# HopperLogger/HopperRender

Hardware: AMD Instinct MI355X
Metric: interpolated frames/sec + ms/flow-calc, 2160p HDR, 1/2/4/8 MI355X (higher is better)
Workload: dtype u16

## Files before the change

### hopperrender_amd/calc.py

```python
import ctypes as C

import numpy as np

from . import capi

BlendedFrame = 2
WarpedFrame12, WarpedFrame21, HSVFlow, GreyFlow, SideBySide1, SideBySide2 = 0, 1, 3, 4, 5, 6


def _ptr(a):
    if isinstance(a, np.ndarray):
        if not a.flags["C_CONTIGUOUS"]:
            raise ValueError("frame buffers must be C-contiguous")
        return a.ctypes.data_as(C.c_void_p)
    return C.c_void_p(a)


class OpticalFlowCalc:

    is_hdr = False

    def __init__(self, frameHeight, frameWidth, inputStride=0, outputStride=0, deltaScalar=8, neighborScalar=6,
                 blackLevel=0.0, whiteLevel=255.0, maxCalcRes=270, *, device_index=0, iterations=0, blur_radius=0,
                 search_radius=0, flags=0):
# ... 197 lines not shown
        return ms.value

    def profile(self):
        pr = capi.HfProfile()
        capi.check(self._lib.hf_get_profile(self._ctx, C.byref(pr)), self._ctx)
        return {k: getattr(pr, k) for k, _ in pr._fields_}

    def setProfileInterval(self, warp_every, flow_every):
        capi.check(self._lib.hf_set_profile_interval(self._ctx, int(warp_every), int(flow_every)), self._ctx)

    def resetProfile(self):
        capi.check(self._lib.hf_reset_profile(self._ctx), self._ctx)

    def readOffsets(self):
        a = np.empty((2, self.m_opticalFlowFrameHeight, self.m_opticalFlowFrameWidth), dtype=np.int16)
        capi.check(self._lib.hf_read_offsets(self._ctx, _ptr(a)), self._ctx)
        return a

    def readBlurredFlow(self, idx):
        a = np.empty((2, self.m_opticalFlowFrameHeight, self.m_opticalFlowFrameWidth), dtype=np.int16)
        capi.check(self._lib.hf_read_blurred_flow(self._ctx, idx, _ptr(a)), self._ctx)
        return a

    def readPhasePlane(self, ring_slot):
        import ctypes
        n = int(self.phase_plane_bytes)
        a = np.empty(n // 4, dtype=np.uint32)
        done = ctypes.c_int(0)
        capi.check(self._lib.hf_read_phase_plane(self._ctx, ring_slot, _ptr(a), ctypes.byref(done)), self._ctx)
        return a, bool(done.value)

    def writeBlurredFlow(self, idx, flow):
        a = np.ascontiguousarray(flow, dtype=np.int16)
        assert a.shape == (2, self.m_opticalFlowFrameHeight, self.m_opticalFlowFrameWidth)
        capi.check(self._lib.hf_write_blurred_flow(self._ctx, idx, _ptr(a)), self._ctx)

    def deviceRcp(self, values):
        x = np.ascontiguousarray(values, dtype=np.float32)
        y = np.empty_like(x)
        capi.check(self._lib.hf_device_rcp(self._ctx, _ptr(x), _ptr(y), len(x)), self._ctx)
        return y

    def countersEnable(self, on=True):
        capi.check(self._lib.hf_debug_counters_enable(self._ctx, 1 if on else 0), self._ctx)

    def counters(self, reset=False):
        cc = capi.HfDebugCounters()
        capi.check(self._lib.hf_debug_counters_read(self._ctx, C.byref(cc), 1 if reset else 0), self._ctx)
        lv = {}
        for k in range(16):
            if cc.level_window_size[k] and (cc.level_windows[k][0] or cc.level_windows[k][1]):
                lv[int(cc.level_window_size[k])] = {"X": (int(cc.level_windows[k][0]), int(cc.level_reused[k][0])),
                                                     "Y": (int(cc.level_windows[k][1]), int(cc.level_reused[k][1]))}
        return {"warp_workgroups": dict(zip(("staged", "interior_global", "generic"), [int(x) for x in cc.warp_workgroups])), "levels": lv}

    def stats(self):
        s = self._stats()
        return {k: getattr(s, k) for k, _ in s._fields_}

    def close(self):
        if getattr(self, "_ctx", None):
            self._lib.hf_destroy(self._ctx)
            self._ctx = C.c_void_p()

    def __del__(self):
        try:
            self.close()
        except Exception:
            pass


class OpticalFlowCalcSDR(OpticalFlowCalc):
    is_hdr = False


class OpticalFlowCalcHDR(OpticalFlowCalc):
    is_hdr = True


ERROR_TILE_DTYPE = np.dtype([("sse", "<u8"), ("sad", "<u4"), ("max_abs", "<u4")])


def frame_error_maps(raw, n, tiles_x, tiles_y):
    a = np.ascontiguousarray(np.frombuffer(raw, dtype=np.uint8) if isinstance(raw, (bytes, bytearray, memoryview)) else raw).reshape(-1).view(np.uint8)
    need = n * 3 * tiles_y * tiles_x * ERROR_TILE_DTYPE.itemsize
    if a.size < need:
        raise ValueError(f"frame_error_maps: {a.size} bytes, {n} maps of 3 x {tiles_y} x {tiles_x} tiles need {need}")
    return a[:need].view(ERROR_TILE_DTYPE).reshape(n, 3, tiles_y, tiles_x)


class DeviceBuffer:

    def __init__(self, nbytes, device_index=0):
        self._lib = capi.load()
        self.device_index, self.nbytes = device_index, nbytes
        p = C.c_void_p()
        capi.check(self._lib.hf_device_malloc(device_index, nbytes, C.byref(p)))
        self.ptr = p.value

    def upload(self, a):
        a = np.ascontiguousarray(a)
        assert a.nbytes <= self.nbytes
        capi.check(self._lib.hf_memcpy_h2d(self.device_index, C.c_void_p(self.ptr), _ptr(a), a.nbytes))

    def download(self, dtype, count=None):
        dt = np.dtype(dtype)
        n = count if count is not None else self.nbytes // dt.itemsize
# ... 154 lines not shown
```

### hopperrender_amd/capi.py

```python
import ctypes as C
import os

from . import build as _build

HF_FLAG_ASYNC = 0x1
HF_FLAG_NO_GRAPH = 0x2
HF_FLAG_PROFILE = 0x4
HF_FLAG_NO_LAZY_ARGMIN = 0x8
HF_FLAG_DUAL_STREAM = 0x40
HF_FLAG_NO_FUSED_WARP = 0x80
HF_FLAG_NO_TIMING = 0x200
HF_FLAG_BATCH_NORMAL_PRIORITY = 0x800
HF_FLAG_BATCH_EAGER_PLANES = 0x1000
HF_FLAG_NO_SAD_REUSE = 0x2000
HF_FLAG_SAD_REUSE_ALWAYS = 0x4000
HF_FLAG_PLANAR_IN = 0x8000
HF_FLAG_PLANAR_OUT = 0x10000
HF_FLAG_BATCH_PLANAR_IN = 0x20000
HF_FLAG_BATCH_PLANAR_OUT = 0x40000
HF_FLAG_BATCH_AUTO_DEFERRED = 0x80000
HF_MAX_PERIOD_OUTPUTS = 6
HF_MAX_PERIOD_OUTPUTS_WIDE = 24
HF_MAX_ERROR_PAIRS = 192
HF_ERROR_SLOTS = 256
# ... 22 lines not shown
                ("first_output", C.c_int64), ("n_outputs", C.c_int64), ("blend_at_start", C.c_double)]


class HfHostioConfig(C.Structure):
    _fields_ = [("struct_size", C.c_uint32), ("in_ring", C.c_int32), ("out_ring", C.c_int32), ("frame_output_mode", C.c_int32),
                ("scene_change_threshold", C.c_int32), ("reserved", C.c_int32), ("source_frame_time", C.c_int64),
                ("target_frame_time", C.c_int64)]


HF_HOSTIO_FILL_FN = C.CFUNCTYPE(C.c_int, C.c_void_p, C.c_int64, C.c_void_p)
HF_HOSTIO_SINK_FN = C.CFUNCTYPE(C.c_int, C.c_void_p, C.c_int64, C.c_void_p, C.c_int32)


class HfParams(C.Structure):
    _fields_ = [("delta_scalar", C.c_int32), ("neighbor_scalar", C.c_int32), ("black_level", C.c_float),
                ("white_level", C.c_float), ("search_radius", C.c_int32), ("frame_count", C.c_uint32)]


class HfStats(C.Structure):
    _fields_ = [("total_frame_delta", C.c_uint32), ("frame_count", C.c_uint32), ("ofc_calc_time", C.c_double),
                ("ofc_avg_calc_time", C.c_double), ("ofc_peak_calc_time", C.c_double), ("warp_calc_time", C.c_double),
                ("res_scalar", C.c_int32), ("low_width", C.c_int32), ("low_height", C.c_int32),
                ("frame_width", C.c_int32), ("frame_height", C.c_int32), ("input_stride", C.c_int32),
                ("output_stride", C.c_int32), ("iterations", C.c_int32), ("initial_window", C.c_int32),
                ("input_frame_bytes", C.c_uint64), ("output_frame_bytes", C.c_uint64), ("phase_plane_bytes", C.c_uint64),
                ("sad_tables", C.c_int32), ("still_share", C.c_float)]


class HfTimelineRecord(C.Structure):
    _fields_ = [("kernel", C.c_char * 32), ("period", C.c_int32), ("flags", C.c_int32), ("start_ms", C.c_double), ("end_ms", C.c_double),
                ("duration_ms", C.c_double)]


class HfSceneRecord(C.Structure):
    _fields_ = [("frame_count", C.c_uint32), ("total_delta", C.c_uint32), ("kind", C.c_int32), ("average", C.c_int32), ("d1", C.c_int32),
                ("d2", C.c_int32)]


class HfFrameError(C.Structure):
    _fields_ = [("sse", C.c_uint64 * 3), ("sad", C.c_uint64 * 3), ("n_differ", C.c_uint64 * 3), ("count", C.c_uint64 * 3),
                ("max_abs", C.c_uint32 * 3), ("reserved", C.c_uint32)]


class HfFrameSsim(C.Structure):
    _fields_ = [("sum_loss_q32", C.c_uint64 * 3), ("max_loss_q32", C.c_uint64 * 3), ("count", C.c_uint64 * 3)]


class HfErrorTile(C.Structure):
    _fields_ = [("sse", C.c_uint64), ("sad", C.c_uint32), ("max_abs", C.c_uint32)]


class HfDebugCounters(C.Structure):
    _fields_ = [("warp_workgroups", C.c_uint32 * 3), ("reserved", C.c_uint32), ("level_windows", (C.c_uint32 * 2) * 16),
                ("level_reused", (C.c_uint32 * 2) * 16), ("level_window_size", C.c_int32 * 16)]


class HfLiveResources(C.Structure):
    _fields_ = [("device_buffers", C.c_int64), ("pinned_buffers", C.c_int64), ("streams", C.c_int64), ("events", C.c_int64),
                ("graph_execs", C.c_int64)]


class HfProfile(C.Structure):
    _fields_ = [("warp_launches", C.c_uint64), ("warp_ms", C.c_double), ("copy_launches", C.c_uint64),
                ("copy_ms", C.c_double), ("flow_chains", C.c_uint64), ("flow_ms", C.c_double), ("warp_frames", C.c_uint64)]


class HfFilterConfig(C.Structure):
    _fields_ = [("struct_size", C.c_uint32), ("scene_change_threshold", C.c_int32), ("source_frame_time", C.c_int64),
                ("target_frame_time", C.c_int64), ("frame_output_mode", C.c_int32), ("auto_adjust", C.c_int32),
                ("active", C.c_int32), ("reserved", C.c_int32)]


class HfFilterState(C.Structure):
    _fields_ = [("num_int_frames", C.c_int32), ("active", C.c_int32), ("blending_scalar", C.c_double),
                ("total_warp_duration", C.c_double), ("playback_frame_time", C.c_int64),
                ("peak_scene_change_delta", C.c_uint32), ("peak_scene_change_delta2", C.c_uint32),
                ("frame_delta_history", C.c_uint32), ("scene_change_history", C.c_uint32),
                ("average_frame_delta", C.c_int32), ("scene_change_delta1", C.c_int32), ("scene_change_delta2", C.c_int32)]


_vp, _i, _f = C.c_void_p, C.c_int, C.c_float
SIGNATURES = {
    "hf_create": (_i, [C.POINTER(HfConfig), C.POINTER(_vp)]),
    "hf_destroy": (None, [_vp]),
    "hf_last_error": (C.c_char_p, [_vp]),
    "hf_abi_version": (_i, []),
    "hf_select_device": (_i, [C.POINTER(HfDeviceCaps), _i, C.c_uint64, C.c_char_p, C.c_size_t]),
    "hf_get_device": (_i, [_vp]),
    "hf_update_frame": (_i, [_vp, _vp]),
    "hf_calculate_optical_flow": (_i, [_vp]),
    "hf_warp_frames": (_i, [_vp, _f, _i]),
    "hf_copy_frame": (_i, [_vp]),
    "hf_download_frame": (_i, [_vp, _vp]),
    "hf_get_params": (_i, [_vp, C.POINTER(HfParams)]),
    "hf_set_params": (_i, [_vp, C.POINTER(HfParams)]),
    "hf_get_stats": (_i, [_vp, C.POINTER(HfStats)]),
    "hf_update_frame_device": (_i, [_vp, _vp]),
    "hf_update_frame_device_ref": (_i, [_vp, _vp]),
    "hf_update_frame_async": (_i, [_vp, _vp]),
    "hf_download_frame_async": (_i, [_vp, _vp]),
    "hf_wait_flow": (_i, [_vp]),
    "hf_downloads_issued": (C.c_uint64, [_vp]),
    "hf_wait_download": (_i, [_vp, C.c_uint64]),
    "hf_interpolate_period": (_i, [_vp, _vp, _i, C.POINTER(C.c_float), C.POINTER(_vp), _i]),
    "hf_interpolate_period_ex": (_i, [_vp, _vp, _i, C.POINTER(C.c_float), C.POINTER(_vp), _i, _i]),
    "hf_batch_create": (_i, [C.POINTER(_vp), _i, C.POINTER(_vp)]),
    "hf_batch_destroy": (None, [_vp]),
# ... 169 lines not shown
```

### hopperrender_amd/csrc/hf_context.hip

```cpp

#include "hf_ctx.h"

using namespace hfi;

namespace {
thread_local std::string g_create_error;
}

namespace hfi {
std::shared_mutex g_capture_mutex;
std::atomic<int64_t> g_live[kLiveKinds];
}

namespace hfi {

int fail(hf_ctx* c, int code, const char* fmt, ...) {
    char buf[512];
    va_list ap;
    va_start(ap, fmt);
    vsnprintf(buf, sizeof(buf), fmt, ap);
    va_end(ap);
    std::string msg = std::string("[HopperRender] ") + buf;
    if (c) c->err = msg; else g_create_error = msg;
    return code;
// ... 409 lines not shown
    if (int rc = set_device(c)) return rc;
    if (int rc = sync_ctx(c)) return rc;
    HF_HIP(c, hipMemcpyAsync(c->blurred[idx].get(), host_in, 2 * c->plane_elems * sizeof(int16_t), hipMemcpyHostToDevice, c->stream));
    hf::launch_pack_flow(c->g, c->blurred[idx].get(), c->blurred_xy[idx].get(), c->stream);
    HF_HIP(c, hipStreamSynchronize(c->stream));
    return HF_OK;
}

int hf_timer_begin(hf_ctx* c) {
    HF_CHECK_CTX(c);
    if (int rc = set_device(c)) return rc;
    if (int rc = leave_warp_stream(c)) return rc;
    HF_HIP(c, hipEventRecord(c->ev_user0.get(), c->stream));
    return HF_OK;
}

int hf_timer_end(hf_ctx* c, float* elapsed_ms) {
    HF_CHECK_CTX(c);
    if (!elapsed_ms) return fail(c, HF_ERR_INVALID_ARGUMENT, "hf_timer_end: null");
    if (int rc = set_device(c)) return rc;
    if (int rc = leave_warp_stream(c)) return rc;
    HF_HIP(c, hipEventRecord(c->ev_user1.get(), c->stream));
    HF_HIP(c, hipEventSynchronize(c->ev_user1.get()));
    HF_HIP(c, hipEventElapsedTime(elapsed_ms, c->ev_user0.get(), c->ev_user1.get()));
    return HF_OK;
}

int hf_debug_counters_enable(hf_ctx* c, int on) {
    HF_CHECK_CTX(c);
    if (int rc = set_device(c)) return rc;
    if (int rc = sync_ctx(c)) return rc;
    c->graphs.clear();
    if (c->batch) c->batch->graphs.clear();
    if (on) {
        if (!c->counters) HF_HIP(c, alloc_device(c->counters, hf::kCounterWords * sizeof(uint32_t)));
        HF_HIP(c, hipMemsetAsync(c->counters.get(), 0, hf::kCounterWords * sizeof(uint32_t), c->stream));
        return sync_ctx(c);
    }
    c->counters.reset();
    return HF_OK;
}

int hf_debug_counters_read(hf_ctx* c, hf_debug_counters* out, int reset) {
    HF_CHECK_CTX(c);
    if (!out) return fail(c, HF_ERR_INVALID_ARGUMENT, "hf_debug_counters_read: null");
    if (!c->counters) return fail(c, HF_ERR_STATE, "hf_debug_counters_read: hf_debug_counters_enable(ctx, 1) first");
    if (int rc = set_device(c)) return rc;
    if (int rc = sync_ctx(c)) return rc;
    uint32_t w[hf::kCounterWords];
    HF_HIP(c, hipMemcpy(w, c->counters.get(), sizeof(w), hipMemcpyDeviceToHost));
    if (reset) HF_HIP(c, hipMemset(c->counters.get(), 0, sizeof(w)));
    memset(out, 0, sizeof(*out));
    for (int i = 0; i < 3; i++) out->warp_workgroups[i] = w[hf::kCounterWarp + i];
    for (int k = 0; k < 16; k++) {
        for (int ax = 0; ax < 2; ax++) {
            out->level_windows[k][ax] = w[hf::kCounterLevels + 4 * k + 2 * ax];
            out->level_reused[k][ax] = w[hf::kCounterLevels + 4 * k + 2 * ax + 1];
        }
        out->level_window_size[k] = k < (int)c->levels.size() && k < c->last_iterations ? c->levels[(size_t)k].window : 0;
    }
    return HF_OK;
}

int hf_debug_bounds_violations(hf_ctx* c, uint32_t* count, uint32_t first[4], int reset) {
    if (!c || !count) return HF_ERR_INVALID_ARGUMENT;
    if (int rc = set_device(c)) return rc;
    if (hipDeviceSynchronize() != hipSuccess) return fail(c, HF_ERR_HIP, "hf_debug_bounds_violations: hipDeviceSynchronize failed");
    unsigned rec[5] = {0, 0, 0, 0, 0};
    const bool a = hf::dbg_bounds_read_kernels(rec, reset != 0), b = hf::dbg_bounds_read_flow(rec, reset != 0),
               p = hf::dbg_bounds_read_planar(rec, reset != 0), s = hf::dbg_bounds_read_scene(rec, reset != 0),
               m = hf::dbg_bounds_read_metrics(rec, reset != 0);
    if (!a || !b || !p || !s || !m) return fail(c, HF_ERR_STATE, "hf_debug_bounds_violations: this library was built without -DHF_DEBUG_BOUNDS (python -m hopperrender_amd.build --debug-bounds)");
    *count = rec[0];
    if (first) for (int i = 0; i < 4; i++) first[i] = rec[1 + i];
    return HF_OK;
}

int hf_debug_bounds_selftest(hf_ctx* c) {
    if (!c) return HF_ERR_INVALID_ARGUMENT;
    uint32_t before = 0, after = 0, first[4] = {0, 0, 0, 0};
    if (int rc = hf_debug_bounds_violations(c, &before, nullptr, 0)) return rc;
    DevBuf<int> scratch;
    if (alloc_device(scratch, 80 * sizeof(int)) != hipSuccess) return fail(c, HF_ERR_OUT_OF_MEMORY, "hf_debug_bounds_selftest: hipMalloc failed");
    hf::launch_bounds_selftest(scratch.get(), c->stream);
    if (hipStreamSynchronize(c->stream) != hipSuccess) return fail(c, HF_ERR_HIP, "hf_debug_bounds_selftest: launch failed");
    if (int rc = hf_debug_bounds_violations(c, &after, first, 0)) return rc;
    if (after - before != 64u || (before == 0 && first[0] != 999u))
        return fail(c, HF_ERR_STATE, "hf_debug_bounds_selftest: 64 out-of-range indices were issued, %u recorded (first site %u)", after - before, first[0]);
    return HF_OK;
}

int hf_device_rcp(hf_ctx* c, const float* host_in, float* host_out, int n) {
    HF_CHECK_CTX(c);
    if (!host_in || !host_out || n < 1 || n > 32) return fail(c, HF_ERR_INVALID_ARGUMENT, "hf_device_rcp: bad argument");
    if (int rc = set_device(c)) return rc;
    if (int rc = sync_ctx(c)) return rc;
    HF_HIP(c, hipMemcpyAsync(c->d_probe.get(), host_in, n * sizeof(float), hipMemcpyHostToDevice, c->stream));
    hf::launch_rcp_probe(c->d_probe.get(), c->d_probe.get() + 32, n, c->stream);
    HF_HIP(c, hipMemcpyAsync(host_out, c->d_probe.get() + 32, n * sizeof(float), hipMemcpyDeviceToHost, c->stream));
    HF_HIP(c, hipStreamSynchronize(c->stream));
    return HF_OK;
}

__global__ void clock_probe_kernel(unsigned long long ticks, unsigned long long* out) {
    const unsigned long long r0 = __builtin_amdgcn_s_memrealtime(), c0 = __builtin_amdgcn_s_memtime();
    unsigned long long r1 = r0;
// ... 95 lines not shown
```

### hopperrender_amd/csrc/hf_kernels.hip

```cpp
#include "hf_kernels.h"
#include "hf_phase_plane.h"
#include "hf_levels.h"
#include <type_traits>

#include <hip/hip_ext.h>

namespace hf {

namespace {

__device__ __forceinline__ int clampi(int v, int lo, int hi) { return min(max(v, lo), hi); }
typedef unsigned nt_uint4 __attribute__((ext_vector_type(4)));
__device__ __forceinline__ void store16_streaming(void* dst, const void* src16) {
    __builtin_nontemporal_store(*(const nt_uint4*)src16, (nt_uint4*)dst);
}
__device__ __forceinline__ unsigned absdiff(unsigned a, unsigned b) { return a > b ? a - b : b - a; }

__device__ __forceinline__ int rel_offset(int layer, int R) {
    const int d = layer - (R >> 1);
    return d > 0 ? d * d : -(d * d);
}

__device__ __forceinline__ int mirror_flow(int pos, int dim) {
    if (pos >= dim) pos = 2 * dim - pos - 1; else if (pos < 0) pos = -pos - 1;
// ... 779 lines not shown
    const int chunk = u % n_chunks, v = u / n_chunks;
    const int member = v / n_blocks, blk = v - member * n_blocks;
    const WarpArgs& a = batch.s[member];
    const int ti0 = chunk * out_chunk, ti1 = min(a.n_out, ti0 + out_chunk);
    if (ti0 >= ti1) return;
    const int tile = blk * wpb + __builtin_amdgcn_readfirstlane(threadIdx.x >> 6);
    if (tile >= n_tiles) return;
    const int trow = tile / wpr, tcol = tile - trow * wpr;
    const int lane = threadIdx.x & 63;
    const int cx0 = (tcol * kWarpTX + (lane & (kWarpTX - 1))) * VEC;
    if (cx0 >= g.W) return;
    if (trow >= y_tiles) {
        const int rg = (trow - y_tiles) * kWarpTY + (lane / kWarpTX);
        if (rg < uv_groups) warp_fast_body<E, GROUP, ROWS, MODE, 1, VB, DW>(g, a, rg * ROWS, cx0, ti0, ti1);
    } else {
        const int rg = trow * kWarpTY + (lane / kWarpTX);
        if (rg < y_groups) warp_fast_body<E, GROUP, ROWS, MODE, 0, VB, DW>(g, a, rg * ROWS, cx0, ti0, ti1);
    }
}


typedef unsigned short ushort2w __attribute__((ext_vector_type(2)));
template <bool MAX>
__device__ __forceinline__ uint32_t pk_mm_u16(uint32_t a, uint32_t b) {
    ushort2w x, y;
    __builtin_memcpy(&x, &a, 4); __builtin_memcpy(&y, &b, 4);
    const ushort2w m = MAX ? __builtin_elementwise_max(x, y) : __builtin_elementwise_min(x, y);
    uint32_t r;
    __builtin_memcpy(&r, &m, 4);
    return r;
}
template <int CTRL>
__device__ __forceinline__ uint32_t dpp_mov(uint32_t v) { return (uint32_t)__builtin_amdgcn_update_dpp(0, (int)v, CTRL, 0xF, 0xF, true); }
template <bool MAX>
__device__ __forceinline__ uint32_t wave_pk_mm_u16(uint32_t v) {
    v = pk_mm_u16<MAX>(v, dpp_mov<0xB1>(v));
    v = pk_mm_u16<MAX>(v, dpp_mov<0x4E>(v));
    v = pk_mm_u16<MAX>(v, dpp_mov<0x141>(v));
    v = pk_mm_u16<MAX>(v, dpp_mov<0x140>(v));
    const uint32_t r0 = (uint32_t)__builtin_amdgcn_readlane((int)v, 0), r1 = (uint32_t)__builtin_amdgcn_readlane((int)v, 16),
                   r2 = (uint32_t)__builtin_amdgcn_readlane((int)v, 32), r3 = (uint32_t)__builtin_amdgcn_readlane((int)v, 48);
    return pk_mm_u16<MAX>(pk_mm_u16<MAX>(r0, r1), pk_mm_u16<MAX>(r2, r3));
}

constexpr int kExtX = 64, kExtY = 64;
constexpr int kWgCells = 64;

template <int NW>
struct WgShared {
    uint2 tab[kMaxWarpOutputs][kWgCells];
    uint32_t bounds[NW][4];
    int state[NW];
    int item[NW];
};

template <typename E, int MODE, int CZ, int NW, int ROWS>
__device__ __forceinline__ void warp_wg_body(const Geom& g, const WarpArgs& a, const int tx0, const int ty0, const bool lane_valid, const int wave,
                                             unsigned char* const lds, WgShared<NW>& sh, uint32_t* const counters) {
    constexpr int VEC = 16 / (int)sizeof(E), NDW = 4, CHUNKS = wg_chunks(NW * ROWS / 2), SZ = (int)sizeof(E);
    constexpr int TW = kWarpTX * VEC, TH = NW * kWarpTY * ROWS, NT = 64 * NW;
    constexpr bool need_a = MODE != 1, need_b = MODE != 0;
    const int H = g.H, W = g.W, Si = g.in_stride, So = g.out_stride, rs = g.rs, lw = g.lw, lh = g.lh;
    const int dim_y = CZ ? (H >> 1) : H;
    const int n = a.n_out;
    const unsigned tid = threadIdx.x, lane = tid & 63u;
    const int cx0 = tx0 + (int)(lane & (kWarpTX - 1)) * VEC, cy0 = ty0 + (wave * kWarpTY + (int)(lane / kWarpTX)) * ROWS;
    const uint64_t valid_mask = __builtin_amdgcn_ballot_w64(lane_valid);
    const bool present = valid_mask != 0, full = __builtin_amdgcn_ballot_w64(lane_valid && cx0 + VEC <= W) == ~0ull;

    const int lcw = rs + CZ;
    const int lgx = max(0, ilog2c(TW) - lcw), lgy = max(0, ilog2c(TH) - rs);
    const int lg = lgx + lgy;
    const int cw = min(1 << lcw, TW), ch = min(1 << rs, TH);
    uint32_t lo_a = 0xFFFFFFFFu, hi_a = 0u, lo_b = 0xFFFFFFFFu, hi_b = 0u;
    bool it_ok = lg <= ilog2c(kWgCells), it_in = true;
    {
        const int cell = (int)tid & ((1 << lg) - 1);
        const int cell_x0 = tx0 + ((cell & ((1 << lgx) - 1)) << lcw), cell_y0 = ty0 + ((cell >> lgx) << rs);
        if (it_ok && cell_x0 < W && cell_y0 < dim_y) {
            const int ly = min(CZ ? ((cell_y0 >> rs) << 1) : (cell_y0 >> rs), lh - 1);
            const int lx = min(CZ ? ((cell_x0 >> rs) & ~1) : (cell_x0 >> rs), lw - 1);
            HF_DBG_CHECK(lx >= 0 && ly >= 0 && cell < kWgCells, 210);
            const uint32_t f12 = a.flow_xy[(size_t)ly * lw + lx];
            const int ox12 = (int)(int16_t)(f12 & 0xFFFFu), oy12 = (int)(int16_t)(f12 >> 16);
            const int py = clampi(ly - (oy12 >> rs), 0, lh - 1), px = clampi(lx - (ox12 >> rs), 0, lw - 1);
            const uint32_t f21 = a.flow_xy[(size_t)py * lw + px];
            const int ox21 = (int)(int16_t)(f21 & 0xFFFFu), oy21 = (int)(int16_t)(f21 >> 16);
            auto item = [&](const int dx, const int dy, uint32_t& lo, uint32_t& hi) -> uint32_t {
                const int dxe = CZ ? (dx & ~1) : dx;
                const int x_lo = cell_x0 + dxe, x_hi = x_lo + cw - VEC, y_lo = cell_y0 + dy, y_hi = y_lo + ch - ROWS;
                const int bx_lo = (x_lo + kExtX) * SZ, bx_hi = (x_hi + kExtX) * SZ, by_lo = y_lo + kExtY, by_hi = y_hi + kExtY;
                bool ok = bx_lo >= 0 && bx_hi + 4 * NDW + 4 <= 0xFFFF && by_lo >= 0 && by_hi + ROWS <= 0xFFFF;
                if (CZ) ok = ok && x_hi + VEC <= W - 2;
                it_ok = it_ok && ok;
                it_in = it_in && x_lo >= 1 && x_hi + VEC - 1 + CZ <= W - 2 && y_lo >= 1 && y_hi + ROWS - 1 <= dim_y - 2;
                if (ok) {
                    lo = pk_mm_u16<false>(lo, ((uint32_t)by_lo << 16) | (uint32_t)bx_lo);
                    hi = pk_mm_u16<true>(hi, ((uint32_t)by_hi << 16) | (uint32_t)bx_hi);
                }
                return (uint32_t)dy * 65536u + (uint32_t)(dxe * SZ + (CZ ? (dx & 1) : 0));
            };
            for (int j = (int)tid >> lg; j < n; j += NT >> lg) {
                float s12t = a.s12v[0], s21t = a.s21v[0];
#pragma unroll
                for (int k = 1; k < kMaxWarpOutputs; k++) { s12t = j == k ? a.s12v[k] : s12t; s21t = j == k ? a.s21v[k] : s21t; }
                uint2 w = make_uint2(0u, 0u);
                if (need_a) w.x = item((int)roundf((float)ox12 * s12t), CZ ? (int)roundf((float)oy12 * s12t * 0.5f) : (int)roundf((float)oy12 * s12t), lo_a, hi_a);
                if (need_b) w.y = item(-(int)roundf((float)ox21 * s21t), -(CZ ? (int)roundf((float)oy21 * s21t * 0.5f) : (int)roundf((float)oy21 * s21t)), lo_b, hi_b);
                sh.tab[j][cell] = w;
            }
        }
    }
    {
        const bool ok_all = __builtin_amdgcn_ballot_w64(!it_ok) == 0, in_all = __builtin_amdgcn_ballot_w64(!it_in) == 0;
        uint32_t b0 = 0xFFFFFFFFu, b1 = 0u, b2 = 0xFFFFFFFFu, b3 = 0u;
        if (need_a) { b0 = wave_pk_mm_u16<false>(lo_a); b1 = wave_pk_mm_u16<true>(hi_a); }
        if (need_b) { b2 = wave_pk_mm_u16<false>(lo_b); b3 = wave_pk_mm_u16<true>(hi_b); }
        const uint32_t mine = lane == 0 ? b0 : lane == 1 ? b1 : lane == 2 ? b2 : b3;
        if (lane < 4) sh.bounds[wave][lane] = mine;
        if (lane == 0) { sh.state[wave] = !present ? 2 : full ? 1 : 0; sh.item[wave] = (ok_all ? 1 : 0) | (in_all ? 2 : 0); }
    }
    __syncthreads();
    bool wg_ok = true, wg_in = true;
    uint32_t m0 = 0xFFFFFFFFu, m1 = 0u, m2 = 0xFFFFFFFFu, m3 = 0u;
#pragma unroll
    for (int w = 0; w < NW; w++) {
        wg_ok = wg_ok && sh.state[w] != 0 && (sh.item[w] & 1) != 0;
        wg_in = wg_in && (sh.item[w] & 2) != 0;
        m0 = pk_mm_u16<false>(m0, sh.bounds[w][0]); m1 = pk_mm_u16<true>(m1, sh.bounds[w][1]);
        m2 = pk_mm_u16<false>(m2, sh.bounds[w][2]); m3 = pk_mm_u16<true>(m3, sh.bounds[w][3]);
    }
    const bool runs_ok = __builtin_amdgcn_readfirstlane((int)wg_ok) != 0;
    wg_in = __builtin_amdgcn_readfirstlane((int)wg_in) != 0;
    int cmin_a = 0, ymin_a = 0, C_a = 1, R_a = 0, cmin_b = 0, ymin_b = 0, C_b = 1, R_b = 0;
    if (runs_ok) {
        const uint32_t la = (uint32_t)__builtin_amdgcn_readfirstlane((int)m0), ha = (uint32_t)__builtin_amdgcn_readfirstlane((int)m1);
        const uint32_t lb = (uint32_t)__builtin_amdgcn_readfirstlane((int)m2), hb = (uint32_t)__builtin_amdgcn_readfirstlane((int)m3);
        if (need_a) {
            cmin_a = (int)(la & 0xFFFFu) >> 4; ymin_a = (int)(la >> 16);
            C_a = (int)(((ha & 0xFFFCu) + 4u * NDW + 3u) >> 4) - cmin_a + 1; R_a = (int)(ha >> 16) + ROWS - 1 - ymin_a + 1;
        }
        if (need_b) {
            cmin_b = (int)(lb & 0xFFFFu) >> 4; ymin_b = (int)(lb >> 16);
            C_b = (int)(((hb & 0xFFFCu) + 4u * NDW + 3u) >> 4) - cmin_b + 1; R_b = (int)(hb >> 16) + ROWS - 1 - ymin_b + 1;
        }
        wg_ok = ((R_a * C_a + 63) & ~63) <= CHUNKS && ((R_b * C_b + 63) & ~63) <= CHUNKS && C_a <= 64 && C_b <= 64;
    }
    wg_ok = __builtin_amdgcn_readfirstlane((int)wg_ok) != 0;
    const uint32_t base = ((uint32_t)(cy0 + kExtY) << 16) | (uint32_t)((cx0 + kExtX) * SZ);
    const int ci = (((cy0 - ty0) >> rs) << lgx) | ((cx0 - tx0) >> lcw);
    HF_DBG_CHECK(!wg_ok || (ci >= 0 && ci < kWgCells), 211);
    if (counters && threadIdx.x == 0) atomicAdd(counters + kCounterWarp + (wg_ok ? 0 : (runs_ok && wg_in && full) ? 1 : 2), 1u);
    if (!wg_ok) {
        if (runs_ok && wg_in && full) {
            const unsigned pitch_g = (unsigned)Si * (unsigned)SZ;
            const unsigned plane_g = (unsigned)dim_y * pitch_g;
            const __amdgpu_buffer_rsrc_t rsrcA = __builtin_amdgcn_make_buffer_rsrc((void*)((const E*)a.frame12 + (size_t)CZ * H * Si), 0, (int)plane_g, 0x00020000);
            const __amdgpu_buffer_rsrc_t rsrcB = __builtin_amdgcn_make_buffer_rsrc((void*)((const E*)a.frame21 + (size_t)CZ * H * Si), 0, (int)plane_g, 0x00020000);
            const Levels lvg = make_levels(a.black, a.white);
            const size_t out_g = (size_t)CZ * H * So + (size_t)cy0 * So + cx0;
            for (int j = 0; j < n; j++) {
                WarpSrc<E, VEC, ROWS, 1> S;
                const uint2 d = sh.tab[j][ci];
                if (need_a) {
                    const uint32_t w = base + d.x, wb = w & 0xFFFFu, odd = CZ ? (wb & 1u) : 0u;
                    const unsigned o = __umul24((w >> 16) - kExtY, pitch_g) + (CZ ? (wb & ~1u) : wb) - (unsigned)(kExtX * SZ);
                    HF_DBG_CHECK((o & ~3u) + 4u * (NDW + 1) + (ROWS - 1) * pitch_g <= plane_g, 10);
#pragma unroll
                    for (int r = 0; r < ROWS; r++) S.ra[r][0] = get_run_buf<E, VEC, CZ>(rsrcA, o + (unsigned)r * pitch_g, odd, plane_g);
                }
                if (need_b) {
                    const uint32_t w = base + d.y, wb = w & 0xFFFFu, odd = CZ ? (wb & 1u) : 0u;
                    const unsigned o = __umul24((w >> 16) - kExtY, pitch_g) + (CZ ? (wb & ~1u) : wb) - (unsigned)(kExtX * SZ);
                    HF_DBG_CHECK((o & ~3u) + 4u * (NDW + 1) + (ROWS - 1) * pitch_g <= plane_g, 11);
#pragma unroll
                    for (int r = 0; r < ROWS; r++) S.rb[r][0] = get_run_buf<E, VEC, CZ>(rsrcB, o + (unsigned)r * pitch_g, odd, plane_g);
                }
                warp_finish<E, VEC, ROWS, MODE, CZ, 16>(S, a.s12v[j], a.s21v[j], (E*)a.outv[j] + out_g, So, ROWS, lvg);
            }
        } else if (lane_valid) {
#pragma unroll
            for (int r = 0; r < ROWS; r += 2)
                if (cy0 + r < dim_y) warp_fast_body<E, VEC, 2, MODE, CZ, 16, true>(g, a, cy0 + r, cx0, 0, n);
        }
        return;
    }

    const unsigned pitch_b = (unsigned)Si * (unsigned)SZ;
    const unsigned plane_bytes = (unsigned)dim_y * pitch_b;
    const E* __restrict__ A = (const E*)a.frame12 + (size_t)CZ * H * Si;
    const E* __restrict__ B = (const E*)a.frame21 + (size_t)CZ * H * Si;
    typedef __attribute__((address_space(3))) void* lds_ptr;
    auto stage = [&](const void* plane, const int cmin, const int ymin, const int C, const int R, unsigned char* const win, auto AUXC) {
        constexpr int AUX = decltype(AUXC)::value;
        const __amdgpu_buffer_rsrc_t rsrc = __builtin_amdgcn_make_buffer_rsrc(const_cast<void*>(plane), 0, (int)plane_bytes, 0x00020000);
        const unsigned magic = ((1u << 20) + (unsigned)C - 1u) / (unsigned)C;
        const int nq = R * C;
#pragma unroll
        for (int i = 0; i < (CHUNKS + 64 * NW - 1) / (64 * NW); i++) {
            const int q0 = (i * NW + wave) * 64;
            if (q0 < nq) {
                const unsigned q = (unsigned)q0 + lane;
                const unsigned row = (q * magic) >> 20, col = q - __umul24(row, (unsigned)C);
                if (wg_in) {
                    const unsigned off = __umul24((unsigned)(ymin - kExtY) + row, pitch_b) + ((unsigned)cmin + col) * 16u - (unsigned)(kExtX * SZ);
                    HF_DBG_CHECK(q >= (unsigned)nq || (size_t)off + 16 <= (size_t)plane_bytes, 212);
                    __builtin_amdgcn_raw_ptr_buffer_load_lds(rsrc, (lds_ptr)(win + (size_t)q0 * 16), 16, off, 0, 0, AUX);
                } else {
                    const int y = mirror_warp_bl(ymin - kExtY + (int)row, dim_y);
                    const int x0 = (cmin + (int)col) * VEC - kExtX;
                    const unsigned rowoff = __umul24((unsigned)y, pitch_b);
                    const bool zone = x0 < 1 || (!CZ && x0 + VEC - 1 > W - 2);
                    if (!zone) {
                        HF_DBG_CHECK(q >= (unsigned)nq || (size_t)rowoff + (size_t)(x0 * SZ) + 16 <= (size_t)plane_bytes, 213);
                        __builtin_amdgcn_raw_ptr_buffer_load_lds(rsrc, (lds_ptr)(win + (size_t)q0 * 16), 16, rowoff + (unsigned)(x0 * SZ), 0, 0, AUX);
                    } else {
                        __attribute__((aligned(16))) E v[VEC];
#pragma unroll
                        for (int k = 0; k < VEC; k++) {
                            const int xs = mirror_warp_bl(x0 + k, W);
                            const unsigned eo = rowoff + (unsigned)((CZ ? (xs & ~1) + ((x0 + k) & 1) : xs) * SZ);
                            HF_DBG_CHECK(eo + SZ <= plane_bytes, 12);
                            if constexpr (SZ == 2) v[k] = (E)__builtin_amdgcn_raw_buffer_load_b16(rsrc, eo, 0, 0);
                            else v[k] = (E)__builtin_amdgcn_raw_buffer_load_b8(rsrc, eo, 0, 0);
                        }
                        *(uint4*)(win + (size_t)q * 16) = *(const uint4*)v;
                    }
                }
            }
        }
    };
    if (need_a) stage(A, cmin_a, ymin_a, C_a, R_a, lds, std::integral_constant<int, 2>{});
    if (need_b) stage(B, cmin_b, ymin_b, C_b, R_b, lds + CHUNKS * 16, std::integral_constant<int, 0>{});
    __builtin_amdgcn_s_waitcnt(0x0F70);
    __syncthreads();
    if (!full) return;

    const Levels lv = make_levels(a.black, a.white);
    using Src = WarpSrc<E, VEC, ROWS, 1>;
    auto lds_run = [&](const unsigned char* p8, const unsigned off, const unsigned odd) {
        const uint32_t* p = (const uint32_t*)p8;
        uint32_t w[NDW + 1];
#pragma unroll
        for (int k = 0; k <= NDW; k++) w[k] = p[k];
        return run_from_dwords<E, VEC, CZ>(w, off, odd);
    };
    const unsigned rowb_a = (unsigned)C_a * 16u, rowb_b = (unsigned)C_b * 16u;
    const unsigned char* const win_a = lds - (unsigned)(ymin_a * C_a + cmin_a) * 16u;
    const unsigned char* const win_b = lds + CHUNKS * 16 - (unsigned)(ymin_b * C_b + cmin_b) * 16u;
    const unsigned out_off = (unsigned)(((size_t)CZ * H * So + (size_t)cy0 * So + cx0) * SZ);
    const unsigned out_pitch = (unsigned)So * (unsigned)SZ;
    const int out_bytes = (int)((size_t)(H + (H >> 1)) * So * SZ);
#pragma unroll 1
    for (int j = 0; j < n; j++) {
        {
            Src S;
            const uint2 d = sh.tab[j][ci];
            if (need_a) {
                const uint32_t w = base + d.x, wb = w & 0xFFFFu, odd = CZ ? (wb & 1u) : 0u, off = CZ ? (wb & ~1u) : wb;
                const unsigned char* p = win_a + __umul24(w >> 16, rowb_a) + (off & ~3u);
                HF_DBG_CHECK(p >= lds && p + (ROWS - 1) * rowb_a + 4 * NDW + 4 <= lds + CHUNKS * 16, 13);
#pragma unroll
                for (int r = 0; r < ROWS; r++) S.ra[r][0] = lds_run(p + (unsigned)r * rowb_a, off, odd);
            }
            if (need_b) {
                const uint32_t w = base + d.y, wb = w & 0xFFFFu, odd = CZ ? (wb & 1u) : 0u, off = CZ ? (wb & ~1u) : wb;
                const unsigned char* p = win_b + __umul24(w >> 16, rowb_b) + (off & ~3u);
                HF_DBG_CHECK(p >= lds + CHUNKS * 16 && p + (ROWS - 1) * rowb_b + 4 * NDW + 4 <= lds + 2 * CHUNKS * 16, 14);
#pragma unroll
                for (int r = 0; r < ROWS; r++) S.rb[r][0] = lds_run(p + (unsigned)r * rowb_b, off, odd);
            }
            const __amdgpu_buffer_rsrc_t rsrc_out = __builtin_amdgcn_make_buffer_rsrc(a.outv[j], 0, out_bytes, 0x00020000);
            warp_finish_to<E, VEC, ROWS, MODE, CZ, 16>(S, a.s12v[j], a.s21v[j], ROWS, lv, [&](const int r, const E* v) {
                __builtin_amdgcn_raw_buffer_store_b128(*(const buf_v4*)v, rsrc_out, out_off, (unsigned)r * out_pitch, 2 );
            });
        }
    }
}

static_assert(sizeof(Geom) + sizeof(WarpBatchArgs) + sizeof(PlaneOut) <= 4096, "kernel arguments of warp_wg_kernel (a launch carries at most 4 KB)");
static_assert(sizeof(WarpArgs) == 168, "hf_kernels.h kMaxWarpBatch is sized for 168-byte members");


template <typename E, int MODE, int NW, int ROWS>
__global__ __launch_bounds__(64 * NW) void warp_wg_kernel(const Geom g, const WarpBatchArgs batch, const PlaneOut po) {
    constexpr int VEC = 16 / (int)sizeof(E);
    const int y_groups = (g.H + ROWS - 1) / ROWS;
    extern __shared__ __attribute__((aligned(16))) unsigned char wg_windows[];
    __shared__ WgShared<NW> sh;
    const int uv_groups = ((g.H >> 1) + ROWS - 1) / ROWS;
    const int wpr = (g.W + kWarpTX * VEC - 1) / (kWarpTX * VEC);
    const int y_tiles = (y_groups + kWarpTY - 1) / kWarpTY, uv_tiles = (uv_groups + kWarpTY - 1) / kWarpTY;
    const int yb = (y_tiles + NW - 1) / NW, ub = (uv_tiles + NW - 1) / NW;
    const int per_sr = wpr * 3 + po.blocks;
    const int n_blocks = wg_blocks_per_member(wpr, yb, ub, po.blocks);
    const int total = n_blocks * batch.n;
    const int per_band = (total + 7) >> 3;
    const int u = (int)(blockIdx.x & 7) * per_band + (int)(blockIdx.x >> 3);
    if (u >= total) return;
    const int member = (int)fastdiv((uint32_t)u, po.per_member), blk = u - member * n_blocks;
    const WarpArgs& a = batch.s[member];
    const int srow = (int)fastdiv((uint32_t)blk, po.per_sr);
    int r = blk - srow * per_sr;
    if (r < po.blocks) {
        if (!a.plane21) return;
        constexpr int LR = 2 * NW * kWarpTY * ROWS;
        const int cgs = (g.W >> g.rs) >> 2;
        const int task = r * (64 * NW) + (int)threadIdx.x;
        const int lr = task / cgs, cg = task - lr * cgs;
        const int y = srow * LR + lr;
        if (lr >= LR || y >= g.H) return;
        if (sizeof(E) == 2 && g.rs == 3) plane_fast_task<E, 3, 1>((const E*)a.frame21, a.plane21, g.H, g.W, g.in_stride, po.pl, y >> 1, cg, y & 1);
        else plane_fast_task<E, 4, 1>((const E*)a.frame21, a.plane21, g.H, g.W, g.in_stride, po.pl, y >> 1, cg, y & 1);
        return;
    }
    r -= po.blocks;
    const int k = (int)fastdiv((uint32_t)r, po.wpr), tcol = r - k * wpr;
    const bool chroma = k == 2;
    const int brow = chroma ? srow : 2 * srow + k;
    if (brow >= (chroma ? ub : yb)) return;
    const int wave = __builtin_amdgcn_readfirstlane(threadIdx.x >> 6), lane = threadIdx.x & 63;
    const int trow = brow * NW + wave;
    const int tx0 = tcol * kWarpTX * VEC, ty0 = brow * NW * kWarpTY * ROWS;
    const int cx0 = tx0 + (lane & (kWarpTX - 1)) * VEC;
    const int rg = trow * kWarpTY + (lane / kWarpTX);
    const bool lane_valid = trow < (chroma ? uv_tiles : y_tiles) && cx0 < g.W && rg < (chroma ? uv_groups : y_groups);
    if (chroma) warp_wg_body<E, MODE, 1, NW, ROWS>(g, a, tx0, ty0, lane_valid, wave, wg_windows, sh, po.counters);
    else warp_wg_body<E, MODE, 0, NW, ROWS>(g, a, tx0, ty0, lane_valid, wave, wg_windows, sh, po.counters);
}
// ... 213 lines not shown
```

### include/hopperflow_diag.h

```cpp
#ifndef HOPPERFLOW_DIAG_H
#define HOPPERFLOW_DIAG_H

#include "hopperflow.h"

#ifdef __cplusplus
extern "C" {
#endif

typedef struct hf_timeline_record {
    char kernel[32];
    int32_t period;
    int32_t flags;
    double start_ms;
    double end_ms;
    double duration_ms;
} hf_timeline_record;
int hf_batch_timeline_enable(hf_batch* batch, int max_launches, int skip_periods);
int hf_batch_timeline_read(hf_batch* batch, hf_timeline_record* out, int capacity, int* n_records);
uint64_t hf_batch_timeline_dropped(const hf_batch* batch);

typedef struct hf_debug_counters {
    uint32_t warp_workgroups[3];
    uint32_t reserved;
    uint32_t level_windows[16][2];
    uint32_t level_reused[16][2];
    int32_t level_window_size[16];
} hf_debug_counters;
int hf_debug_counters_enable(hf_ctx* ctx, int on);
int hf_debug_counters_read(hf_ctx* ctx, hf_debug_counters* out, int reset);

int hf_debug_bounds_violations(hf_ctx* ctx, uint32_t* count, uint32_t first[4], int reset);
int hf_debug_bounds_selftest(hf_ctx* ctx);
int hf_device_rcp(hf_ctx* ctx, const float* host_in, float* host_out, int n);

int hf_clock_probe(int device_index, int duration_us, double* shader_mhz);
int hf_hbm_copy_probe(int device_index, size_t bytes, int repeats, double* read_plus_write_GBps);

typedef struct hf_live_resources {
    int64_t device_buffers;
    int64_t pinned_buffers;
    int64_t streams;
    int64_t events;
    int64_t graph_execs;
} hf_live_resources;
int hf_debug_live_resources(hf_live_resources* out);

int hf_timer_begin(hf_ctx* ctx);
int hf_timer_end(hf_ctx* ctx, float* elapsed_ms);

int hf_planar_convert_device(hf_ctx* ctx, int to_planar, const void* device_src, void* device_dst);

#ifdef __cplusplus
}
#endif
#endif
```

Measured before the change: 98200.

## Restage warp windows in LDS groups when the combined window overflows shared memory

Workgroups whose union of source windows did not fit the LDS budget used to fall back to the interior-global or generic warp path. Now such a workgroup is still staged if the packed window sizes fit a 64-chunk-aligned budget. Otherwise the outputs are split into consecutive groups whose windows each fit, and each group is staged and warped in turn with a barrier between groups. The goal is to keep more workgroups on the LDS-staged path. The cost is extra per-wave reductions to compute the group windows, more shared state, and repeated staging and syncs for multi-group workgroups. New debug counters report how often each restaging mode is taken.

```diff
diff --git a/hopperrender_amd/calc.py b/hopperrender_amd/calc.py
--- a/hopperrender_amd/calc.py
+++ b/hopperrender_amd/calc.py
@@ -273,7 +273,8 @@
             if cc.level_window_size[k] and (cc.level_windows[k][0] or cc.level_windows[k][1]):
                 lv[int(cc.level_window_size[k])] = {"X": (int(cc.level_windows[k][0]), int(cc.level_reused[k][0])),
                                                      "Y": (int(cc.level_windows[k][1]), int(cc.level_reused[k][1]))}
-        return {"warp_workgroups": dict(zip(("staged", "interior_global", "generic"), [int(x) for x in cc.warp_workgroups])), "levels": lv}
+        return {"warp_workgroups": dict(zip(("staged", "interior_global", "generic"), [int(x) for x in cc.warp_workgroups])),
+                "warp_restaged": dict(zip(("shared_budget", "groups"), [int(x) for x in cc.warp_restaged])), "levels": lv}
 
     def stats(self):
         s = self._stats()
diff --git a/hopperrender_amd/capi.py b/hopperrender_amd/capi.py
--- a/hopperrender_amd/capi.py
+++ b/hopperrender_amd/capi.py
@@ -98,7 +98,7 @@
 
 class HfDebugCounters(C.Structure):
     _fields_ = [("warp_workgroups", C.c_uint32 * 3), ("reserved", C.c_uint32), ("level_windows", (C.c_uint32 * 2) * 16),
-                ("level_reused", (C.c_uint32 * 2) * 16), ("level_window_size", C.c_int32 * 16)]
+                ("level_reused", (C.c_uint32 * 2) * 16), ("level_window_size", C.c_int32 * 16), ("warp_restaged", C.c_uint32 * 2)]
 
 
 class HfLiveResources(C.Structure):
diff --git a/hopperrender_amd/csrc/hf_context.hip b/hopperrender_amd/csrc/hf_context.hip
--- a/hopperrender_amd/csrc/hf_context.hip
+++ b/hopperrender_amd/csrc/hf_context.hip
@@ -485,6 +485,7 @@
     if (reset) HF_HIP(c, hipMemset(c->counters.get(), 0, sizeof(w)));
     memset(out, 0, sizeof(*out));
     for (int i = 0; i < 3; i++) out->warp_workgroups[i] = w[hf::kCounterWarp + i];
+    for (int i = 0; i < 2; i++) out->warp_restaged[i] = w[hf::kCounterWarp + 3 + i];
     for (int k = 0; k < 16; k++) {
         for (int ax = 0; ax < 2; ax++) {
             out->level_windows[k][ax] = w[hf::kCounterLevels + 4 * k + 2 * ax];
diff --git a/hopperrender_amd/csrc/hf_kernels.hip b/hopperrender_amd/csrc/hf_kernels.hip
--- a/hopperrender_amd/csrc/hf_kernels.hip
+++ b/hopperrender_amd/csrc/hf_kernels.hip
@@ -855,6 +855,7 @@
     uint32_t bounds[NW][4];
     int state[NW];
     int item[NW];
+    uint32_t groups[NW][kMaxWarpOutputs][4];
 };
 
 template <typename E, int MODE, int CZ, int NW, int ROWS>
@@ -954,6 +955,73 @@
     const int ci = (((cy0 - ty0) >> rs) << lgx) | ((cx0 - tx0) >> lcw);
     HF_DBG_CHECK(!wg_ok || (ci >= 0 && ci < kWgCells), 211);
     if (counters && threadIdx.x == 0) atomicAdd(counters + kCounterWarp + (wg_ok ? 0 : (runs_ok && wg_in && full) ? 1 : 2), 1u);
+
+    auto window_of = [&](const uint32_t lo, const uint32_t hi, int& cmin, int& ymin, int& C, int& R) {
+        cmin = (int)(lo & 0xFFFFu) >> 4; ymin = (int)(lo >> 16);
+        C = (int)(((hi & 0xFFFCu) + 4u * NDW + 3u) >> 4) - cmin + 1; R = (int)(hi >> 16) + ROWS - 1 - ymin + 1;
+    };
+    auto chunks64 = [](const int C, const int R) { return (R * C + 63) & ~63; };
+    auto fits_shared = [&](const uint32_t lo_1, const uint32_t hi_1, const uint32_t lo_2, const uint32_t hi_2) {
+        int cm, ym, C1 = 1, R1 = 0, C2 = 1, R2 = 0;
+        if (need_a) window_of(lo_1, hi_1, cm, ym, C1, R1);
+        if (need_b) window_of(lo_2, hi_2, cm, ym, C2, R2);
+        return chunks64(C1, R1) + chunks64(C2, R2) <= 2 * CHUNKS && C1 <= 64 && C2 <= 64;
+    };
+    int how = 0;
+    uint32_t gmask = 0;
+    if (runs_ok && !wg_ok) {
+        if (chunks64(C_a, R_a) + chunks64(C_b, R_b) <= 2 * CHUNKS && C_a <= 64 && C_b <= 64) {
+            how = 1;
+        } else if (n > 1) {
+            const int gc = (int)lane;
+            const int gc_x0 = tx0 + ((gc & ((1 << lgx) - 1)) << lcw), gc_y0 = ty0 + ((gc >> lgx) << rs);
+            const bool gc_valid = gc < (1 << lg) && gc_x0 < W && gc_y0 < dim_y;
+            const uint32_t gc_base = ((uint32_t)(gc_y0 + kExtY) << 16) | (uint32_t)((gc_x0 + kExtX) * SZ);
+            const uint32_t span = ((uint32_t)(ch - ROWS) << 16) | (uint32_t)((cw - VEC) * SZ);
+            uint32_t u0 = 0xFFFFFFFFu, u1 = 0u, u2 = 0xFFFFFFFFu, u3 = 0u;
+            int ng = 0;
+            bool each_fits = true;
+#pragma unroll 1
+            for (int k = 0; k < n; k++) {
+                uint2 d = make_uint2(0u, 0u);
+                if (gc_valid) d = sh.tab[k][gc];
+                uint32_t b0 = 0xFFFFFFFFu, b1 = 0u, b2 = 0xFFFFFFFFu, b3 = 0u;
+                if (need_a) {
+                    const uint32_t lo = (gc_base + d.x) & (CZ ? ~1u : ~0u);
+                    b0 = wave_pk_mm_u16<false>(gc_valid ? lo : 0xFFFFFFFFu); b1 = wave_pk_mm_u16<true>(gc_valid ? lo + span : 0u);
+                }
+                if (need_b) {
+                    const uint32_t lo = (gc_base + d.y) & (CZ ? ~1u : ~0u);
+                    b2 = wave_pk_mm_u16<false>(gc_valid ? lo : 0xFFFFFFFFu); b3 = wave_pk_mm_u16<true>(gc_valid ? lo + span : 0u);
+                }
+                const uint32_t t0 = pk_mm_u16<false>(u0, b0), t1 = pk_mm_u16<true>(u1, b1), t2 = pk_mm_u16<false>(u2, b2), t3 = pk_mm_u16<true>(u3, b3);
+                if (fits_shared(t0, t1, t2, t3)) {
+                    u0 = t0; u1 = t1; u2 = t2; u3 = t3;
+                } else {
+                    if (k > 0) {
+                        const uint32_t mine = lane == 0 ? u0 : lane == 1 ? u1 : lane == 2 ? u2 : u3;
+                        if (lane < 4) sh.groups[wave][ng][lane] = mine;
+                        ng++;
+                        gmask |= 1u << (k - 1);
+                    }
+                    each_fits = each_fits && fits_shared(b0, b1, b2, b3);
+                    u0 = b0; u1 = b1; u2 = b2; u3 = b3;
+                }
+            }
+            {
+                const uint32_t mine = lane == 0 ? u0 : lane == 1 ? u1 : lane == 2 ? u2 : u3;
+                if (lane < 4) sh.groups[wave][ng][lane] = mine;
+            }
+            gmask |= 1u << (n - 1);
+            if (each_fits) how = 2;
+        }
+    }
+    how = __builtin_amdgcn_readfirstlane(how);
+    gmask = (uint32_t)__builtin_amdgcn_readfirstlane((int)gmask);
+    if (how) {
+        wg_ok = true;
+        if (counters && threadIdx.x == 0) atomicAdd(counters + kCounterWarp + 2 + how, 1u);
+    }
     if (!wg_ok) {
         if (runs_ok && wg_in && full) {
             const unsigned pitch_g = (unsigned)Si * (unsigned)SZ;
@@ -999,10 +1067,9 @@
         const __amdgpu_buffer_rsrc_t rsrc = __builtin_amdgcn_make_buffer_rsrc(const_cast<void*>(plane), 0, (int)plane_bytes, 0x00020000);
         const unsigned magic = ((1u << 20) + (unsigned)C - 1u) / (unsigned)C;
         const int nq = R * C;
-#pragma unroll
-        for (int i = 0; i < (CHUNKS + 64 * NW - 1) / (64 * NW); i++) {
-            const int q0 = (i * NW + wave) * 64;
-            if (q0 < nq) {
+#pragma unroll 1
+        for (int q0 = wave * 64; q0 < nq; q0 += 64 * NW) {
+            {
                 const unsigned q = (unsigned)q0 + lane;
                 const unsigned row = (q * magic) >> 20, col = q - __umul24(row, (unsigned)C);
                 if (wg_in) {
@@ -1033,12 +1100,6 @@
             }
         }
     };
-    if (need_a) stage(A, cmin_a, ymin_a, C_a, R_a, lds, std::integral_constant<int, 2>{});
-    if (need_b) stage(B, cmin_b, ymin_b, C_b, R_b, lds + CHUNKS * 16, std::integral_constant<int, 0>{});
-    __builtin_amdgcn_s_waitcnt(0x0F70);
-    __syncthreads();
-    if (!full) return;
-
     const Levels lv = make_levels(a.black, a.white);
     using Src = WarpSrc<E, VEC, ROWS, 1>;
     auto lds_run = [&](const unsigned char* p8, const unsigned off, const unsigned odd) {
@@ -1048,36 +1109,57 @@
         for (int k = 0; k <= NDW; k++) w[k] = p[k];
         return run_from_dwords<E, VEC, CZ>(w, off, odd);
     };
-    const unsigned rowb_a = (unsigned)C_a * 16u, rowb_b = (unsigned)C_b * 16u;
-    const unsigned char* const win_a = lds - (unsigned)(ymin_a * C_a + cmin_a) * 16u;
-    const unsigned char* const win_b = lds + CHUNKS * 16 - (unsigned)(ymin_b * C_b + cmin_b) * 16u;
     const unsigned out_off = (unsigned)(((size_t)CZ * H * So + (size_t)cy0 * So + cx0) * SZ);
     const unsigned out_pitch = (unsigned)So * (unsigned)SZ;
     const int out_bytes = (int)((size_t)(H + (H >> 1)) * So * SZ);
+    int j0 = 0, gi = 0;
 #pragma unroll 1
-    for (int j = 0; j < n; j++) {
-        {
-            Src S;
-            const uint2 d = sh.tab[j][ci];
-            if (need_a) {
-                const uint32_t w = base + d.x, wb = w & 0xFFFFu, odd = CZ ? (wb & 1u) : 0u, off = CZ ? (wb & ~1u) : wb;
-                const unsigned char* p = win_a + __umul24(w >> 16, rowb_a) + (off & ~3u);
-                HF_DBG_CHECK(p >= lds && p + (ROWS - 1) * rowb_a + 4 * NDW + 4 <= lds + CHUNKS * 16, 13);
-#pragma unroll
-                for (int r = 0; r < ROWS; r++) S.ra[r][0] = lds_run(p + (unsigned)r * rowb_a, off, odd);
-            }
-            if (need_b) {
-                const uint32_t w = base + d.y, wb = w & 0xFFFFu, odd = CZ ? (wb & 1u) : 0u, off = CZ ? (wb & ~1u) : wb;
-                const unsigned char* p = win_b + __umul24(w >> 16, rowb_b) + (off & ~3u);
-                HF_DBG_CHECK(p >= lds + CHUNKS * 16 && p + (ROWS - 1) * rowb_b + 4 * NDW + 4 <= lds + 2 * CHUNKS * 16, 14);
-#pragma unroll
-                for (int r = 0; r < ROWS; r++) S.rb[r][0] = lds_run(p + (unsigned)r * rowb_b, off, odd);
-            }
-            const __amdgpu_buffer_rsrc_t rsrc_out = __builtin_amdgcn_make_buffer_rsrc(a.outv[j], 0, out_bytes, 0x00020000);
-            warp_finish_to<E, VEC, ROWS, MODE, CZ, 16>(S, a.s12v[j], a.s21v[j], ROWS, lv, [&](const int r, const E* v) {
-                __builtin_amdgcn_raw_buffer_store_b128(*(const buf_v4*)v, rsrc_out, out_off, (unsigned)r * out_pitch, 2 );
-            });
-        }
+    for (;;) {
+        int j1 = n;
+        if (how == 2) {
+            const uint32_t gw = sh.groups[wave][gi][lane & 3u];
+            const uint32_t la = (uint32_t)__builtin_amdgcn_readlane((int)gw, 0), ha = (uint32_t)__builtin_amdgcn_readlane((int)gw, 1);
+            const uint32_t lb = (uint32_t)__builtin_amdgcn_readlane((int)gw, 2), hb = (uint32_t)__builtin_amdgcn_readlane((int)gw, 3);
+            if (need_a) window_of(la, ha, cmin_a, ymin_a, C_a, R_a);
+            if (need_b) window_of(lb, hb, cmin_b, ymin_b, C_b, R_b);
+            j1 = j0 + __builtin_ctz(gmask >> j0) + 1;
+        }
+        unsigned char* const lds_b = lds + chunks64(C_a, R_a) * 16;
+        if (need_a) stage(A, cmin_a, ymin_a, C_a, R_a, lds, std::integral_constant<int, 2>{});
+        if (need_b) stage(B, cmin_b, ymin_b, C_b, R_b, lds_b, std::integral_constant<int, 0>{});
+        __builtin_amdgcn_s_waitcnt(0x0F70);
+        __syncthreads();
+        if (full) {
+            const unsigned rowb_a = (unsigned)C_a * 16u, rowb_b = (unsigned)C_b * 16u;
+            const unsigned char* const win_a = lds - (unsigned)(ymin_a * C_a + cmin_a) * 16u;
+            const unsigned char* const win_b = lds_b - (unsigned)(ymin_b * C_b + cmin_b) * 16u;
+#pragma unroll 1
+            for (int j = j0; j < j1; j++) {
+                Src S;
+                const uint2 d = sh.tab[j][ci];
+                if (need_a) {
+                    const uint32_t w = base + d.x, wb = w & 0xFFFFu, odd = CZ ? (wb & 1u) : 0u, off = CZ ? (wb & ~1u) : wb;
+                    const unsigned char* p = win_a + __umul24(w >> 16, rowb_a) + (off & ~3u);
+                    HF_DBG_CHECK(p >= lds && p + (ROWS - 1) * rowb_a + 4 * NDW + 4 <= lds_b, 13);
+#pragma unroll
+                    for (int r = 0; r < ROWS; r++) S.ra[r][0] = lds_run(p + (unsigned)r * rowb_a, off, odd);
+                }
+                if (need_b) {
+                    const uint32_t w = base + d.y, wb = w & 0xFFFFu, odd = CZ ? (wb & 1u) : 0u, off = CZ ? (wb & ~1u) : wb;
+                    const unsigned char* p = win_b + __umul24(w >> 16, rowb_b) + (off & ~3u);
+                    HF_DBG_CHECK(p >= lds_b && p + (ROWS - 1) * rowb_b + 4 * NDW + 4 <= lds_b + chunks64(C_b, R_b) * 16 && lds_b + chunks64(C_b, R_b) * 16 <= lds + 2 * CHUNKS * 16, 14);
+#pragma unroll
+                    for (int r = 0; r < ROWS; r++) S.rb[r][0] = lds_run(p + (unsigned)r * rowb_b, off, odd);
+                }
+                const __amdgpu_buffer_rsrc_t rsrc_out = __builtin_amdgcn_make_buffer_rsrc(a.outv[j], 0, out_bytes, 0x00020000);
+                warp_finish_to<E, VEC, ROWS, MODE, CZ, 16>(S, a.s12v[j], a.s21v[j], ROWS, lv, [&](const int r, const E* v) {
+                    __builtin_amdgcn_raw_buffer_store_b128(*(const buf_v4*)v, rsrc_out, out_off, (unsigned)r * out_pitch, 2 );
+                });
+            }
+        }
+        if (j1 >= n) break;
+        j0 = j1; gi++;
+        __syncthreads();
     }
 }
 
diff --git a/include/hopperflow_diag.h b/include/hopperflow_diag.h
--- a/include/hopperflow_diag.h
+++ b/include/hopperflow_diag.h
@@ -25,6 +25,7 @@
     uint32_t level_windows[16][2];
     uint32_t level_reused[16][2];
     int32_t level_window_size[16];
+    uint32_t warp_restaged[2];
 } hf_debug_counters;
 int hf_debug_counters_enable(hf_ctx* ctx, int on);
 int hf_debug_counters_read(hf_ctx* ctx, hf_debug_counters* out, int reset);
```

Result: no change. 98640 (median of 6 runs) (+0.4%).
